# pirovc/ganon

Measured on AMD Instinct MI355X. Metric: Mreads/s classified (150 bp) + IBF-lookup GB/s vs HBM roofline, higher is better.
Workload: dtype u64

## Files before the change

### ganon_amd/csrc/gn_kernels.hip

```cpp
#include "gn_internal.h"
#include <cstdlib>

#define GN_WAVE 64
#define GN_CAND_LIMIT 128u
#ifndef GN_NARROW_MAX
#define GN_NARROW_MAX 4u
#endif
#define GN_MATCH_CHUNK 256u
#ifndef GN_MATCH_CHUNK_MAX
#define GN_MATCH_CHUNK_MAX 8192u
#endif
#define GN_STAGE_CAP 128u

struct GnRankLut
{
    uint8_t t[256];
    constexpr GnRankLut() : t{}
    {
        for (int i = 0; i < 256; ++i)
            t[i] = 0;
        t['C'] = t['c'] = 1;
        t['G'] = t['g'] = 2;
        t['T'] = t['t'] = t['U'] = t['u'] = 3;
        t['Y'] = t['y'] = 1;
// ... 656 lines not shown
            if (rec.y >= 1)
                s += lds_count(rec.z);
            if (rec.y >= 2)
                s += lds_count(rec.w);
            for (uint32_t x = 2; x < rec.y; ++x)
                s += lds_count(p.tgt_lds[rec.x + x]);
            return s > n ? n : s;
        };
        auto target_count = [&](uint32_t t) -> uint32_t {
            if (p.tgt_off == nullptr)
            {
                const uint32_t s = bin_count(t);
                return s > n ? n : s;
            }
            return rec_count(p.tgt_rec[t]);
        };

        auto emit_hits = [&](bool emit, uint32_t tgt, uint32_t cv, uint32_t& tot, bool direct, gn_match* out) {
            const uint64_t bm = __ballot(emit);
            if (emit)
            {
                const uint32_t o = tot + __popcll(bm & ((1ULL << lane) - 1ULL));
                if (direct)
                {
                    gn_match mt;
                    mt.read   = read;
                    mt.target = tgt;
                    mt.count  = cv;
                    out[o]    = mt;
                }
                else if (o < GN_STAGE_CAP)
                {
                    stage[2 * o]     = tgt;
                    stage[2 * o + 1] = cv;
                }
            }
            tot += (uint32_t)__popcll(bm);
        };
        auto cand_rounds = [&](bool direct, gn_match* out) -> uint32_t {
            uint32_t c[ND];
#pragma unroll
            for (int d = 0; d < ND; ++d)
                c[d] = cand[d];
            uint32_t tot = 0;
            {
                const uint32_t per = (p.n_big + wpr - 1) / wpr;
                const uint32_t lo = min(p.n_big, slice * per), hi = min(p.n_big, lo + per);
                for (uint32_t i0 = lo; i0 < hi; i0 += GN_WAVE)
                {
                    const uint32_t i = i0 + lane;
                    bool           emit = false;
                    uint32_t       tgt = 0, cv = 0;
                    if (i < hi)
                    {
                        const uint32_t t = p.big_list[i];
                        cv               = rec_count(p.tgt_rec[t]);
                        emit             = cv >= T;
                        tgt              = p.tgt_ids ? p.tgt_ids[t] : t;
                    }
                    emit_hits(emit, tgt, cv, tot, direct, out);
                }
            }
            for (;;)
            {
                bool     have = false;
                uint32_t tp   = 0;
#pragma unroll
                for (int d = 0; d < ND; ++d)
                    if (!have && c[d])
                    {
                        have = true;
                        tp   = 32u * d + (uint32_t)__builtin_ctz(c[d]);
                        c[d] &= c[d] - 1;
                    }
                if (__ballot(have) == 0)
                    break;
                bool     emit = false;
                uint32_t tgt = 0, cv = 0;
                if (have)
                {
                    const uint32_t b   = wi * 64 + tp;
                    const uint32_t t   = p.bin_tgt[b];
                    const uint4    rec = p.tgt_rec[t];
                    const uint32_t nbc = rec.y;
                    bool           lowest = true;
                    for (uint32_t x = 0; x < rec.y; ++x)
                    {
                        if (p.tgt_bins[rec.x + x] >= b)
                            break;
                        const uint32_t cx = lds_count(x == 0 ? rec.z : (x == 1 ? rec.w : p.tgt_lds[rec.x + x]));
                        if (cx * nbc >= T)
                        {
                            lowest = false;
                            break;
                        }
                    }
                    if (lowest)
                    {
                        cv   = rec_count(rec);
                        emit = cv >= T;
                        tgt  = p.tgt_ids ? p.tgt_ids[t] : t;
                    }
                }
                emit_hits(emit, tgt, cv, tot, direct, out);
            }
            return tot;
        };

        uint32_t total    = 0;
        bool     overflow = false;
        if (use_cand)
        {
            total    = cand_rounds(false, nullptr);
            overflow = total > GN_STAGE_CAP;
        }
        else if (n)
            for (uint32_t t0 = t_lo; t0 < t_hi; t0 += 4 * GN_WAVE)
            {
                uint4 rec[4];
                if (p.tgt_off != nullptr)
                {
#pragma unroll
                    for (int u = 0; u < 4; ++u)
                    {
                        const uint32_t t = t0 + u * GN_WAVE + lane;
                        rec[u]           = t < t_hi ? p.tgt_rec[t] : make_uint4(0, 0, 0, 0);
                    }
                }
#pragma unroll
                for (int u = 0; u < 4; ++u)
                {
                    const uint32_t t   = t0 + u * GN_WAVE + lane;
                    uint32_t       c   = 0;
                    bool           hit = false;
                    if (t < t_hi)
                    {
                        if (p.tgt_off != nullptr)
                            c = rec_count(rec[u]);
                        else
                        {
                            c = bin_count(t);
                            c = c > n ? n : c;
                        }
                        hit = c >= T;
                    }
                    const uint64_t bm = __ballot(hit);
                    const uint32_t nb = (uint32_t)__popcll(bm);
                    if (!overflow && total + nb <= GN_STAGE_CAP)
                    {
                        if (hit)
                        {
                            const uint32_t o = total + __popcll(bm & ((1ULL << lane) - 1ULL));
                            stage[2 * o]     = p.tgt_ids ? p.tgt_ids[t] : t;
                            stage[2 * o + 1] = c;
                        }
                    }
                    else
                        overflow = true;
                    total += nb;
                }
            }
        unsigned long long base = 0;
        if (total)
        {
            if (total > chunk_left)
            {
                const uint32_t need = total > chunk_size ? total : chunk_size;
                chunk_size = chunk_size * 2u <= GN_MATCH_CHUNK_MAX ? chunk_size * 2u : GN_MATCH_CHUNK_MAX;
                unsigned long long nb = 0;
                if (lane == 0)
                    nb = atomicAdd(p.cursor, (unsigned long long)need);
                chunk_base = gn_readlane64(nb, 0);
                chunk_left = need;
            }
            base = chunk_base;
            chunk_base += total;
            chunk_left -= total;
            if (base + total <= p.match_cap)
            {
                if (!overflow)
                {
                    gn_wave_lds_sync();
                    for (uint32_t o = lane; o < total; o += GN_WAVE)
                    {
                        gn_match mt;
                        mt.read   = read;
                        mt.target = stage[2 * o];
                        mt.count  = stage[2 * o + 1];
                        p.matches[base + o] = mt;
                    }
                    gn_wave_lds_sync();
                }
                else if (use_cand)
                    (void)cand_rounds(true, p.matches + base);
                else
                {
                    uint32_t run = 0;
                    for (uint32_t t0 = t_lo; t0 < t_hi; t0 += GN_WAVE)
                    {
                        const uint32_t t   = t0 + lane;
                        uint32_t       c   = 0;
                        bool           hit = false;
                        if (t < t_hi)
                        {
                            c   = target_count(t);
                            hit = c >= T;
                        }
                        const uint64_t bm = __ballot(hit);
                        if (hit)
                        {
                            gn_match mt;
                            mt.read   = read;
                            mt.target = p.tgt_ids ? p.tgt_ids[t] : t;
                            mt.count  = c;
                            p.matches[base + run + __popcll(bm & ((1ULL << lane) - 1ULL))] = mt;
                        }
                        run += __popcll(bm);
                    }
                }
            }
        }
        if (lane == 0)
        {
            p.seg_begin[(size_t)read * wpr + slice] = base;
            p.seg_count[(size_t)read * wpr + slice] = total;
        }
    }
    __syncthreads();
    }
}

#define GN_FAST_LIST 512u
#ifndef GN_FAST_WPE_LW1
#define GN_FAST_WPE_LW1 4
#endif
#ifndef GN_FAST_WPE_LW2
#define GN_FAST_WPE_LW2 2
#endif
#ifndef GN_FAST_WPE_LW2_H4
#define GN_FAST_WPE_LW2_H4 3
#endif

constexpr uint32_t GN_FAST_EE_GP_LOG2 = 6;
static_assert((1u << GN_FAST_EE_GP_LOG2) == GN_WAVE, "the EE instances of the fast kernel: one hash group a wave");
template <int HF, int LW, bool EE, bool WIDE = false, bool SCRN = false>
__global__ __launch_bounds__(256) __attribute__((amdgpu_waves_per_eu(EE ? (LW == 1 ? GN_FAST_WPE_LW1 : (HF <= 4 && !WIDE ? GN_FAST_WPE_LW2_H4 : GN_FAST_WPE_LW2)) : 1))) void gn_ibf_count_fast_kernel(GnCountParams p)
{
    extern __shared__ __attribute__((aligned(16))) uint32_t gn_lds[];
    constexpr int      ND   = 2 * LW;
    constexpr int      HFP  = HF <= 4 ? 4 : 8;
    constexpr uint32_t NMAX = 127;
    constexpr bool     SCR  = SCRN && EE && HF == 4 && (LW == 1 || WIDE);
    static_assert(SCR == SCRN, "a screening instance: early exit, four hash functions, 8-byte lanes or the wide build");

    const int      lane  = threadIdx.x & (GN_WAVE - 1);
    const int      wave  = __builtin_amdgcn_readfirstlane((int)(threadIdx.x >> 6));
    const uint32_t wpr   = p.wpr;
    const uint32_t gpl   = SCR ? GN_FAST_EE_GP_LOG2 : p.gp_log2;
    const uint32_t Gp    = 1u << gpl;
    const uint32_t H     = GN_WAVE >> gpl;
    const uint32_t gl    = lane & (Gp - 1);
    const uint32_t hsub  = lane >> gpl;
    uint32_t*      rowtab = gn_lds + (size_t)wave * 128 * HFP;
    uint32_t*      mlist  = gn_lds + (size_t)(blockDim.x >> 6) * 128 * HFP + (size_t)wave * GN_FAST_LIST;

    const uint64_t n_units = (uint64_t)(p.n_reads - p.read_begin) * wpr;
    const uint64_t stride  = (uint64_t)gridDim.x * (blockDim.x >> 6);
    uint64_t       unit    = (uint64_t)blockIdx.x * (blockDim.x >> 6) + wave;
    if (unit >= n_units)
        return;
    const bool     dyn      = p.grab != nullptr && n_units >= 64u * stride;
    const uint64_t dyn_from = stride * 16u;
    uint64_t       chunk_end = unit + 1;
    if (dyn)
    {
        unit *= 16u;
        chunk_end = unit + 16u;
    }
    unsigned long long g_next = 0;
    uint32_t           g_size = 16u;
    auto               ask    = [&](uint64_t from) {
        g_size = from < n_units - n_units / 4u ? 16u : (from < n_units - n_units / 16u ? 8u : 4u);
        if (lane == 0)
            g_next = atomicAdd(p.grab, (unsigned long long)g_size);
    };
    if (dyn)
        ask(unit);
    const uint32_t q0_c = (uint32_t)lane / HF, q1_c = ((uint32_t)lane + GN_WAVE) / HF;
    auto hash_of = [&](uint32_t& q0, uint32_t& q1) {
        if constexpr (!SCR)
        {
            q0 = q0_c;
            q1 = q1_c;
            return;
        }
        uint32_t l = (uint32_t)lane;
        if constexpr (SCR)
            asm volatile("" : "+v"(l));
        q0 = l / HF;
        q1 = (l + GN_WAVE) / HF;
    };
    auto load_meta = [&](uint64_t u, uint32_t& rd, uint32_t& nn, uint64_t& so) {
        rd = p.read_begin + (uint32_t)(u / wpr);
        nn = p.status[rd] == GN_READ_OK ? p.n_hashes[rd] : 0u;
        so = p.slot_off[rd];
    };
    auto load_hashes = [&](uint32_t nn, uint64_t so, uint64_t& h0, uint64_t& h1) {
        h0 = h1 = 0;
        if (nn >= 1 && nn <= NMAX)
        {
            uint32_t q0, q1;
            hash_of(q0, q1);
            if (q0 < nn)
                h0 = p.hashes[so + q0];
            if (q1 < nn)
                h1 = p.hashes[so + q1];
        }
    };
    unsigned long long chunk_base = 0;
    uint32_t           chunk_left = 0, chunk_size = GN_MATCH_CHUNK;
    uint64_t           skipped_bytes = 0;
    uint32_t           n_pre = 0;
    uint32_t read, n;
    uint64_t slot, hA, hB;
    load_meta(unit, read, n, slot);
    load_hashes(n, slot, hA, hB);

    for (;;)
    {
    const uint32_t slice = (uint32_t)(unit - (uint64_t)(read - p.read_begin) * wpr);
    uint64_t unit_n = unit + 1;
    if (unit_n >= chunk_end)
    {
        if (dyn)
        {
            const uint32_t lo32 = (uint32_t)__builtin_amdgcn_readfirstlane((int)(uint32_t)g_next);
            const uint32_t hi32 = (uint32_t)__builtin_amdgcn_readfirstlane((int)(uint32_t)(g_next >> 32));
            unit_n              = dyn_from + (((uint64_t)hi32 << 32) | lo32);
            chunk_end           = unit_n + g_size;
            if (unit_n < n_units)
                ask(unit_n);
        }
        else
        {
            unit_n    = unit + stride;
            chunk_end = unit_n + 1;
        }
    }
    const bool more = unit_n < n_units;
    uint32_t       read_n = 0, n_n = 0;
    uint64_t       slot_n = 0, hA_n = 0, hB_n = 0;
    if (more)
        load_meta(unit_n, read_n, n_n, slot_n);

    if (n > NMAX || n == 0)
    {
        if (lane == 0)
        {
            if (n > NMAX && slice == 0)
                p.work_list_out[atomicAdd(p.work_count_out, 1ULL)] = read;
            p.seg_begin[(size_t)read * wpr + slice] = 0;
            p.seg_count[(size_t)read * wpr + slice] = 0;
        }
        if (!more)
            break;
        load_hashes(n_n, slot_n, hA_n, hB_n);
        unit = unit_n; read = read_n; n = n_n; slot = slot_n; hA = hA_n; hB = hB_n;
        continue;
    }
    const uint32_t  wi      = slice * 64 * LW + gl * LW;
    const bool      col_act = wi < p.W;

    gn_wave_lds_sync();
    uint32_t q0, q1;
    hash_of(q0, q1);
    if ((uint32_t)lane < n * HF)
        rowtab[q0 * HFP + ((uint32_t)lane - q0 * HF)] = gn_ibf_row(hA, (uint32_t)lane - q0 * HF, p.shift, p.S);
    if ((uint32_t)lane + GN_WAVE < n * HF)
        rowtab[q1 * HFP + ((uint32_t)lane + GN_WAVE - q1 * HF)] = gn_ibf_row(hB, (uint32_t)lane + GN_WAVE - q1 * HF, p.shift, p.S);
    for (uint32_t idx = (uint32_t)lane + 2 * GN_WAVE; idx < n * HF; idx += GN_WAVE)
    {
        const uint32_t q = idx / HF, i = idx - q * HF;
        rowtab[q * HFP + i] = gn_ibf_row(p.hashes[slot + q], i, p.shift, p.S);
    }
    gn_wave_lds_sync();

    uint32_t nib[ND][4];
    uint32_t byt[ND][4][2];
#pragma unroll
    for (int d = 0; d < ND; ++d)
#pragma unroll
        for (int j = 0; j < 4; ++j)
        {
            nib[d][j]    = 0;
            byt[d][j][0] = 0;
            byt[d][j][1] = 0;
        }
    uint32_t acc_n = 0;
    auto spill_nibbles = [&]() {
#pragma unroll
        for (int d = 0; d < ND; ++d)
#pragma unroll
            for (int j = 0; j < 4; ++j)
            {
                byt[d][j][0] += nib[d][j] & 0x0F0F0F0Fu;
                byt[d][j][1] += (nib[d][j] >> 4) & 0x0F0F0F0Fu;
                nib[d][j] = 0;
            }
    };

    const uint32_t iters = (n + H - 1) / H;
    uint32_t T = (uint32_t)(uint64_t)ceil(__dmul_rn((double)n, p.rel_cutoff));
    if (T == 0)
        T = 1;
    uint32_t chk1 = 0xFFFFFFFFu, chk2 = 0xFFFFFFFFu;
    if (EE && p.early_exit && T >= 2)
    {
        uint32_t c = (2 * (n - T + 1) + H - 1) / H;
        if (c < 1)
            c = 1;
        if (c + 2 <= iters)
        {
            chk1 = p.early_exit == 3 ? c : (c > 1 ? c - 1 : c);
            chk2 = p.early_exit >= 2 && p.early_exit != 3 ? iters - 2 : c + 2;
        }
    }
    uint32_t ds = 0;
    if constexpr (SCR)
    {
        if (p.early_exit && T >= 2)
        {
            ds = (p.screen[n >> 2] >> (8u * (n & 3u))) & 0xFFu;
            if (ds > n || ds + T <= n)
                ds = 0;
        }
    }
    const uint32_t wi_ld = col_act ? wi : 0u;
    auto load_row = [&](uint32_t row, auto& R, int i) {
        const uint64_t* ptr = p.rows + ((uint64_t)row * p.W + wi_ld);
        if constexpr (LW == 2)
        {
            typedef uint32_t gn_u32x4 __attribute__((ext_vector_type(4)));
            const gn_u32x4* p4 = reinterpret_cast<const gn_u32x4*>(ptr);
            const gn_u32x4  v  = *p4;
            R.m[i][0] = v.x;
            R.m[i][1] = v.y;
            R.m[i][2] = v.z;
            R.m[i][3] = v.w;
        }
        else
        {
            const uint2 v = *reinterpret_cast<const uint2*>(ptr);
            R.m[i][0] = v.x;
            R.m[i][1] = v.y;
        }
    };
    bool scr = SCR && ds != 0;
    auto issue = [&](uint32_t it, GnRowRegs<HF, LW>& R) {
        uint32_t q = it * H + hsub;
        q          = q < n ? q : n - 1;
        uint32_t row[HF];
#pragma unroll
        for (int i = 0; i < HF; ++i)
        {
            uint32_t idx = q * HFP + (uint32_t)i;
            if constexpr (SCR)
            {
                const uint32_t qs = 2 * it + (uint32_t)(i >> 1) < ds ? 2 * it + (uint32_t)(i >> 1) : 2 * it;
                idx               = scr ? qs * HFP + (uint32_t)(i & 1) : idx;
            }
            row[i] = rowtab[idx];
        }
#pragma unroll
        for (int i = 0; i < HF; ++i)
            load_row(row[i], R, i);
    };
    auto consume = [&](const GnRowRegs<HF, LW>& R, uint32_t it) {
        if (SCR && scr)
        {
            const uint32_t on = col_act ? 0xFFFFFFFFu : 0u, on2 = 2 * it + 1 < ds ? on : 0u;
#pragma unroll
            for (int d = 0; d < ND; ++d)
            {
                const uint32_t a = R.m[0][d] & R.m[1][d] & on, b = R.m[2 % HF][d] & R.m[3 % HF][d] & on2;
#pragma unroll
                for (int j = 0; j < 4; ++j)
                    nib[d][j] += ((a >> j) & 0x11111111u) + ((b >> j) & 0x11111111u);
            }
            acc_n += 2;
            if (acc_n >= 14)
            {
                spill_nibbles();
                acc_n = 0;
            }
            return;
        }
        const uint32_t on = (col_act && it * H + hsub < n) ? 0xFFFFFFFFu : 0u;
#pragma unroll
        for (int d = 0; d < ND; ++d)
        {
            uint32_t a = R.m[0][d] & on;
#pragma unroll
            for (int i = 1; i < HF; ++i)
                a &= R.m[i][d];
#pragma unroll
            for (int j = 0; j < 4; ++j)
                nib[d][j] += (a >> j) & 0x11111111u;
        }
        if (++acc_n == 15)
        {
            spill_nibbles();
            acc_n = 0;
        }
    };
    uint32_t sm[ND];
#pragma unroll
    for (int d = 0; d < ND; ++d)
        sm[d] = 0;
    auto survivors = [&](uint32_t tval) -> uint32_t {
        const uint32_t Kt = (0x80u - tval) * 0x01010101u;
        uint32_t any_t = 0;
#pragma unroll
        for (int d = 0; d < ND; ++d)
        {
            uint32_t m = 0;
#pragma unroll
            for (int j = 0; j < 4; ++j)
#pragma unroll
                for (int pp = 0; pp < 2; ++pp)
                {
                    const uint32_t g = (byt[d][j][pp] + Kt) & 0x80808080u;
                    any_t |= g;
                    m |= (g >> 7) << (4 * pp + j);
                }
            sm[d] = m;
        }
        if (__ballot(any_t != 0) == 0)
            return 0u;
        uint32_t c = 0;
#pragma unroll
        for (int d = 0; d < ND; ++d)
            c += (uint32_t)__popc(sm[d]);
        for (int off = 32; off > 0; off >>= 1)
            c += __shfl_xor(c, off);
        return c;
    };
    auto survey = [&](uint32_t done) -> uint32_t {
        if (acc_n)
        {
            spill_nibbles();
            acc_n = 0;
        }
        return survivors(T - (n - done));
    };
    bool     dead    = false;
    bool     narrow  = false;
    uint32_t fetched = iters;
    bool     finish   = false;
    bool     aborted  = false;
    uint32_t scr_rows = 0;
    for (;;)
    {
        GnRowRegs<HF, LW> A, Bq;
        const uint32_t    its     = SCR && scr ? (ds + 1) >> 1 : iters;
        const uint32_t    c1      = SCR && scr ? 0xFFFFFFFFu : chk1, c2 = chk2;
        uint32_t          it      = 0;
        bool              drained = false;
        issue(0, A);
        for (; it + 2 < its; it += 2)
        {
            if (EE && narrow)
                break;
            issue(it + 1, Bq);
            consume(A, it);
            if constexpr (EE)
            {
                const uint32_t done = it + 1;
                if (done >= c1 && done <= c2)
                {
                    const uint32_t left = survey(done);
                    if (left == 0)
                    {
                        dead    = true;
                        fetched = done + 1;
                        break;
                    }
                    if (left <= GN_NARROW_MAX && (done > c1 || (done > 2 && survivors(done - 1) == left)))
                    {
                        consume(Bq, it + 1);
                        narrow  = true;
                        fetched = it + 2;
                        drained = true;
                        break;
                    }
                }
            }
            issue(it + 2, A);
            consume(Bq, it + 1);
            if constexpr (EE)
            {
                const uint32_t done = it + 2;
                if (done >= c1 && done <= c2)
                {
                    const uint32_t left = survey(done);
                    if (left == 0)
                    {
                        dead    = true;
                        fetched = done + 1;
                        break;
                    }
                    if (left <= GN_NARROW_MAX)
                        narrow = true;
                }
            }
        }
        if (!dead && !drained)
        {
            const bool two = !(EE && narrow) && it + 1 < its;
            if (two)
                issue(it + 1, Bq);
            consume(A, it);
            if (two)
                consume(Bq, it + 1);
            if (EE && narrow)
                fetched = it + 1;
        }
        if (!(SCR && scr))
            break;
        scr                 = false;
        scr_rows            = 2 * ds;
        const uint32_t left = survey(ds);
        if (left == 0)
            dead = true;
        else if (left <= GN_NARROW_MAX)
            finish = true;
        if (dead || finish)
            break;
        aborted = true;
#pragma unroll
        for (int d = 0; d < ND; ++d)
#pragma unroll
            for (int j = 0; j < 4; ++j)
            {
                byt[d][j][0] = 0;
                byt[d][j][1] = 0;
            }
    }
    uint32_t narrow_loads = 0;
    if (EE && (narrow || (SCR && finish)))
    {
        constexpr uint32_t QPC = GN_WAVE / HF;
        uint64_t           grp = 0;
#pragma unroll
        for (uint32_t q = 0; q < QPC; ++q)
            grp |= 1ULL << (q * HF);
        const uint32_t l_q = (uint32_t)lane / HF, l_i = (uint32_t)lane - l_q * HF;
        const uint32_t q_from = SCR && finish ? 0u : fetched;
        uint32_t       any_sm = 0;
#pragma unroll
        for (int d = 0; d < ND; ++d)
            any_sm |= sm[d];
        uint64_t lm = __ballot(any_sm != 0);
        while (lm)
        {
            const int L = __builtin_ctzll(lm);
            lm &= lm - 1;
#pragma unroll
            for (int d = 0; d < ND; ++d)
            {
                uint32_t mb = (uint32_t)__builtin_amdgcn_readlane((int)sm[d], L);
                while (mb)
                {
                    const uint32_t bit = (uint32_t)__builtin_ctz(mb);
                    mb &= mb - 1;
                    const uint32_t tp   = 32u * d + bit;
                    const uint32_t word = slice * 64 * LW + (uint32_t)L * LW + (tp >> 6);
                    const uint32_t sh   = tp & 63u;
                    uint32_t       add  = 0;
                    uint32_t       q_known = 0;
                    uint32_t       q_to    = n;
                    bool           probe   = false;
                    if (SCR && finish)
                    {
                        uint32_t c2 = 0;
#pragma unroll
                        for (int j = 0; j < 4; ++j)
#pragma unroll
                            for (int pp = 0; pp < 2; ++pp)
                                if ((bit & 3u) == (uint32_t)j && ((bit >> 2) & 1u) == (uint32_t)pp)
                                    c2 = byt[d][j][pp];
                        c2      = ((uint32_t)__builtin_amdgcn_readlane((int)c2, L) >> (8u * (bit >> 3))) & 0xFFu;
                        q_known = ds;
                        if (c2 != ds)
                        {
                            probe = true;
                            q_to  = ds;
                        }
                    }
                    for (;;)
                    {
                        add = 0;
                        for (uint32_t q0 = q_from; q0 < q_to; q0 += QPC)
                        {
                            const uint32_t q  = q0 + l_q;
                            bool           on = false;
                            if (l_q < QPC && q < q_to)
                            {
                                if (SCR && l_i < 2 && q < q_known)
                                    on = true;
                                else
                                {
                                    const uint32_t row = rowtab[q * HFP + l_i];
                                    on = (p.rows[(uint64_t)row * p.W + word] >> sh) & 1ULL;
                                }
                            }
                            const uint64_t bm  = __ballot(on);
                            uint64_t       all = bm;
#pragma unroll
                            for (int i = 1; i < HF; ++i)
                                all &= bm >> i;
                            add += (uint32_t)__popcll(all & grp);
                        }
                        narrow_loads += (q_to - q_from) * HF - 2 * q_known;
                        if (!(SCR && probe))
                            break;
                        probe = false;
                        if (add + (n - ds) < T)
                        {
                            add = 0;
                            break;
                        }
                        q_known = 0;
                        q_to    = n;
                    }
                    const uint32_t inc  = add << (8u * (bit >> 3));
                    const uint32_t keep = SCR && finish ? ~(0xFFu << (8u * (bit >> 3))) : 0xFFFFFFFFu;
#pragma unroll
                    for (int j = 0; j < 4; ++j)
#pragma unroll
                        for (int pp = 0; pp < 2; ++pp)
                            if ((bit & 3u) == (uint32_t)j && ((bit >> 2) & 1u) == (uint32_t)pp && lane == L)
                                byt[d][j][pp] = (byt[d][j][pp] & keep) + inc;
                }
            }
        }
    }
    if (slice * 64 * LW < p.W)
    {
        const uint32_t wcol = p.W - slice * 64 * LW < 64u * LW ? p.W - slice * 64 * LW : 64u * LW;
        if constexpr (!SCR)
        {
            if (dead || narrow)
            {
                const uint32_t got  = fetched < n ? fetched : n;
                const uint64_t full = (uint64_t)(n - got) * HF * wcol * 8ull;
                const uint64_t part = (uint64_t)narrow_loads * 128ull;
                skipped_bytes += full - part;
            }
        }
        else if (dead || narrow || finish)
        {
            const uint32_t got  = fetched < n ? fetched : n;
            const uint32_t rows = SCR && scr_rows && !aborted ? scr_rows : got * HF;
            const uint64_t full = (uint64_t)(n * HF - rows) * wcol * 8ull;
            const uint64_t part = (uint64_t)narrow_loads * 128ull;
            skipped_bytes += full - part;
        }
        if (SCR && aborted)
            skipped_bytes -= (uint64_t)scr_rows * wcol * 8ull;
    }

    if (more)
        load_hashes(n_n, slot_n, hA_n, hB_n);

    uint32_t Kc  = (0x80u - T) * 0x01010101u;
    uint32_t any = 0;
    if (!dead)
    {
        if (acc_n)
            spill_nibbles();
#pragma unroll
        for (int d = 0; d < ND; ++d)
#pragma unroll
            for (int j = 0; j < 4; ++j)
#pragma unroll
                for (int pp = 0; pp < 2; ++pp)
                {
                    uint32_t x = byt[d][j][pp];
                    for (uint32_t off = Gp; off < GN_WAVE; off <<= 1)
                        x += __shfl_xor(x, (int)off);
                    byt[d][j][pp] = x;
                    any |= (x + Kc) & 0x80808080u;
                }
    }
    const bool owner = hsub == 0 && col_act;
    uint64_t   hm    = dead ? 0ull : __ballot(owner && any != 0);
    if (p.pre_mode && __popcll(hm) > 6)
    {
        auto any_ge = [&](uint32_t v) -> bool {
            const uint32_t K = (0x80u - v) * 0x01010101u;
            uint32_t       a = 0;
#pragma unroll
            for (int d = 0; d < ND; ++d)
#pragma unroll
                for (int j = 0; j < 4; ++j)
#pragma unroll
                    for (int pp = 0; pp < 2; ++pp)
                        a |= byt[d][j][pp] + K;
            return __ballot(owner && (a & 0x80808080u) != 0) != 0;
        };
        uint32_t lo = T, hi = n;
        while (lo < hi)
        {
            const uint32_t mid = (lo + hi + 1) >> 1;
            if (any_ge(mid))
                lo = mid;
            else
                hi = mid - 1;
        }
        const uint32_t t2 = gn_pf_threshold(lo, p.pre_mode == 1 ? T : 0u, p.pre_rel);
        if (t2 > T && t2 <= lo)
        {
            const uint32_t K2 = (0x80u - t2) * 0x01010101u;
            auto in_range = [&](uint32_t v, bool count) -> uint32_t {
                const uint32_t K1 = (0x80u - (v + 1u)) * 0x01010101u;
                uint32_t       a = 0;
#pragma unroll
                for (int d = 0; d < ND; ++d)
#pragma unroll
                    for (int j = 0; j < 4; ++j)
#pragma unroll
                        for (int pp = 0; pp < 2; ++pp)
                        {
                            const uint32_t e = ((byt[d][j][pp] + Kc) & ~(byt[d][j][pp] + K1)) & 0x80808080u;
                            a = count ? a + (uint32_t)__popc(e) : (a | e);
                        }
                return a;
            };
            const uint32_t below = owner ? in_range(t2 - 1u, true) : 0u;
            if (__ballot(below != 0))
            {
                uint32_t a = T, b = t2 - 1u;
                while (a < b)
                {
                    const uint32_t mid = (a + b) >> 1;
                    if (__ballot(owner && in_range(mid, false) != 0))
                        b = mid;
                    else
                        a = mid + 1u;
                }
                if (lane == 0)
                    p.seg_min[(size_t)read * wpr + slice] = a;
                n_pre += below;
                Kc  = K2;
                any = 0;
#pragma unroll
                for (int d = 0; d < ND; ++d)
#pragma unroll
                    for (int j = 0; j < 4; ++j)
#pragma unroll
                        for (int pp = 0; pp < 2; ++pp)
                            any |= (byt[d][j][pp] + Kc) & 0x80808080u;
                hm = __ballot(owner && any != 0);
            }
        }
    }
    uint32_t       total = 0;
    unsigned long long base = 0;
    if (hm)
    {
        uint32_t hit[ND];
        uint32_t mine = 0;
#pragma unroll
        for (int d = 0; d < ND; ++d)
        {
            hit[d] = 0;
            if (owner && any)
            {
#pragma unroll
                for (int j = 0; j < 4; ++j)
#pragma unroll
                    for (int pp = 0; pp < 2; ++pp)
                        hit[d] |= ((((byt[d][j][pp] + Kc) & 0x80808080u) >> 7) << (4 * pp + j));
            }
            mine += __popc(hit[d]);
        }
        uint32_t my_off = 0;
        if (__popcll(hm) <= 6)
        {
            uint64_t rem = hm;
            while (rem)
            {
                const uint32_t L = (uint32_t)__builtin_ctzll(rem);
                rem &= rem - 1;
                const uint32_t c = (uint32_t)__builtin_amdgcn_readlane((int)mine, (int)L);
                if ((uint32_t)lane == L)
                    my_off = total;
                total += c;
            }
        }
        else
        {
            uint32_t x = mine;
#pragma unroll
            for (int off = 1; off < GN_WAVE; off <<= 1)
            {
                const uint32_t y = (uint32_t)__shfl_up((int)x, off);
                if (lane >= off)
                    x += y;
            }
            my_off = x - mine;
            total  = (uint32_t)__builtin_amdgcn_readlane((int)x, GN_WAVE - 1);
        }
        if (total > chunk_left)
        {
            const uint32_t need = total > chunk_size ? total : chunk_size;
                chunk_size = chunk_size * 2u <= GN_MATCH_CHUNK_MAX ? chunk_size * 2u : GN_MATCH_CHUNK_MAX;
            unsigned long long nb = 0;
            if (lane == 0)
                nb = atomicAdd(p.cursor, (unsigned long long)need);
            chunk_base = gn_readlane64(nb, 0);
            chunk_left = need;
        }
        base = chunk_base;
        chunk_base += total;
        chunk_left -= total;
        const bool fits = base + total <= p.match_cap;
        if (__popcll(hm) > 6)
        {
            const uint8_t* tabb   = reinterpret_cast<const uint8_t*>(rowtab);
            const bool     listed = total <= GN_FAST_LIST;
            if (p.emit_probe & 128u)
                goto emitted;
            gn_match*      out    = p.matches + base + my_off;
            uint32_t       k      = 0;
#pragma unroll
            for (int d = 0; d < ND; ++d)
            {
                gn_wave_lds_sync();
                if (owner && any)
                {
#pragma unroll
                    for (int j = 0; j < 4; ++j)
#pragma unroll
                        for (int pp = 0; pp < 2; ++pp)
                            rowtab[(uint32_t)lane * 8u + (uint32_t)(j * 2 + pp)] = byt[d][j][pp];
                }
                gn_wave_lds_sync();
                uint32_t mbits = (fits && owner && any) ? hit[d] : 0u;
                while (mbits)
                {
                    const uint32_t b = (uint32_t)__builtin_ctz(mbits);
                    mbits &= mbits - 1;
                    const uint32_t cnt = tabb[(uint32_t)lane * 32u + (((b & 3u) << 1) + ((b >> 2) & 1u)) * 4u + (b >> 3)];
                    const uint32_t bin = (uint32_t)(gl * LW) * 64u + 32u * (uint32_t)d + b;
                    if (listed)
                        mlist[my_off + k] = (bin << 8) | cnt;
                    else
                    {
                        gn_match mt;
                        mt.read   = read;
                        mt.target = slice * 64u * LW * 64u + bin;
                        mt.count  = cnt;
                        out[k]    = mt;
                    }
                    ++k;
                }
            }
            gn_wave_lds_sync();
            if (listed && fits && !(p.emit_probe & 64u))
            {
                gn_match* seg = p.matches + base;
                for (uint32_t m = (uint32_t)lane; m < total; m += GN_WAVE)
                {
                    const uint32_t e = mlist[m];
                    gn_match       mt;
                    mt.read   = read;
                    mt.target = slice * 64u * LW * 64u + (e >> 8);
                    mt.count  = e & 0xFFu;
                    seg[m] = mt;
                }
                gn_wave_lds_sync();
            }
        }
        else if (fits && owner && any)
        {
            gn_match* out = p.matches + base + my_off;
            uint32_t  before = 0;
#pragma unroll
            for (int d = 0; d < ND; ++d)
            {
#pragma unroll
                for (int j = 0; j < 4; ++j)
#pragma unroll
                    for (int pp = 0; pp < 2; ++pp)
                    {
                        uint32_t hbits = (byt[d][j][pp] + Kc) & 0x80808080u;
                        while (hbits)
                        {
                            const uint32_t y = (uint32_t)__builtin_ctz(hbits) >> 3;
                            hbits &= hbits - 1;
                            const uint32_t bitpos = 8 * y + 4 * pp + j;
                            gn_match mt;
                            mt.read   = read;
                            mt.target = wi * 64 + 32 * d + bitpos;
                            mt.count  = (byt[d][j][pp] >> (8 * y)) & 0xFFu;
                            out[before + __popc(hit[d] & ((1u << bitpos) - 1u))] = mt;
                        }
                    }
                before += __popc(hit[d]);
            }
        }
    }
emitted:
    if (lane == 0)
    {
        p.seg_begin[(size_t)read * wpr + slice] = base;
        p.seg_count[(size_t)read * wpr + slice] = total;
    }
    if (!more)
        break;
    unit = unit_n; read = read_n; n = n_n; slot = slot_n; hA = hA_n; hB = hB_n;
    }
    if (lane == 0 && skipped_bytes)
// ... 244 lines not shown
```

Baseline: 267.6.

## Defer next-read metadata load and unroll narrow-phase row probes by two

In the SCR variant, the next work unit's metadata load now happens after the first row fetch is issued, instead of before the main loop. This moves the metadata latency behind the IBF row loads. The first row-register fetch is hoisted out of the retry loop and re-issued only after an abort. The narrow-phase verification loop now handles two query groups per iteration, keeping two independent row loads in flight before the ballots. The cost is more live registers and changed control flow around the aborted-retry path.

```diff
diff --git a/ganon_amd/csrc/gn_kernels.hip b/ganon_amd/csrc/gn_kernels.hip
--- a/ganon_amd/csrc/gn_kernels.hip
+++ b/ganon_amd/csrc/gn_kernels.hip
@@ -982,7 +982,8 @@
     };
     auto load_meta = [&](uint64_t u, uint32_t& rd, uint32_t& nn, uint64_t& so) {
         rd = p.read_begin + (uint32_t)(u / wpr);
-        nn = p.status[rd] == GN_READ_OK ? p.n_hashes[rd] : 0u;
+        const uint32_t nh = p.n_hashes[rd];
+        nn = p.status[rd] == GN_READ_OK ? nh : 0u;
         so = p.slot_off[rd];
     };
     auto load_hashes = [&](uint32_t nn, uint64_t so, uint64_t& h0, uint64_t& h1) {
@@ -1030,7 +1031,8 @@
     const bool more = unit_n < n_units;
     uint32_t       read_n = 0, n_n = 0;
     uint64_t       slot_n = 0, hA_n = 0, hB_n = 0;
-    if (more)
+    constexpr bool META_LATE = SCR;
+    if (!META_LATE && more)
         load_meta(unit_n, read_n, n_n, slot_n);
 
     if (n > NMAX || n == 0)
@@ -1044,6 +1046,8 @@
         }
         if (!more)
             break;
+        if (META_LATE)
+            load_meta(unit_n, read_n, n_n, slot_n);
         load_hashes(n_n, slot_n, hA_n, hB_n);
         unit = unit_n; read = read_n; n = n_n; slot = slot_n; hA = hA_n; hB = hB_n;
         continue;
@@ -1239,14 +1243,16 @@
     bool     finish   = false;
     bool     aborted  = false;
     uint32_t scr_rows = 0;
+    GnRowRegs<HF, LW> A, Bq;
+    issue(0, A);
+    if (META_LATE && more)
+        load_meta(unit_n, read_n, n_n, slot_n);
     for (;;)
     {
-        GnRowRegs<HF, LW> A, Bq;
         const uint32_t    its     = SCR && scr ? (ds + 1) >> 1 : iters;
         const uint32_t    c1      = SCR && scr ? 0xFFFFFFFFu : chk1, c2 = chk2;
         uint32_t          it      = 0;
         bool              drained = false;
-        issue(0, A);
         for (; it + 2 < its; it += 2)
         {
             if (EE && narrow)
@@ -1325,6 +1331,7 @@
                 byt[d][j][0] = 0;
                 byt[d][j][1] = 0;
             }
+        issue(0, A);
     }
     uint32_t narrow_loads = 0;
     if (EE && (narrow || (SCR && finish)))
@@ -1380,26 +1387,24 @@
                     for (;;)
                     {
                         add = 0;
-                        for (uint32_t q0 = q_from; q0 < q_to; q0 += QPC)
+                        for (uint32_t q0 = q_from; q0 < q_to; q0 += 2 * QPC)
                         {
-                            const uint32_t q  = q0 + l_q;
-                            bool           on = false;
-                            if (l_q < QPC && q < q_to)
+                            const uint32_t qa = q0 + l_q, qb = qa + QPC;
+                            const bool     ina = l_q < QPC && qa < q_to, inb = l_q < QPC && qb < q_to;
+                            uint64_t       wa = ~0ULL, wb = ~0ULL;
+                            if (ina && !(SCR && l_i < 2 && qa < q_known))
+                                wa = p.rows[(uint64_t)rowtab[qa * HFP + l_i] * p.W + word];
+                            if (inb && !(SCR && l_i < 2 && qb < q_known))
+                                wb = p.rows[(uint64_t)rowtab[qb * HFP + l_i] * p.W + word];
+                            const uint64_t bma = __ballot(ina && ((wa >> sh) & 1ULL)), bmb = __ballot(inb && ((wb >> sh) & 1ULL));
+                            uint64_t       alla = bma, allb = bmb;
+#pragma unroll
+                            for (int i = 1; i < HF; ++i)
                             {
-                                if (SCR && l_i < 2 && q < q_known)
-                                    on = true;
-                                else
-                                {
-                                    const uint32_t row = rowtab[q * HFP + l_i];
-                                    on = (p.rows[(uint64_t)row * p.W + word] >> sh) & 1ULL;
-                                }
+                                alla &= bma >> i;
+                                allb &= bmb >> i;
                             }
-                            const uint64_t bm  = __ballot(on);
-                            uint64_t       all = bm;
-#pragma unroll
-                            for (int i = 1; i < HF; ++i)
-                                all &= bm >> i;
-                            add += (uint32_t)__popcll(all & grp);
+                            add += (uint32_t)__popcll(alla & grp) + (uint32_t)__popcll(allb & grp);
                         }
                         narrow_loads += (q_to - q_from) * HF - 2 * q_known;
                         if (!(SCR && probe))
```

New measurement: 278.1, median of 6. 1.04x the previous value.
